# ETH3D/dataset-pipeline

Hardware: AMD Instinct MI355X
Metric: ICP correspondences/sec (higher is better)
Workload: dtype f32 (f64 accumulation); 1 GPU; ICPScanAligner 2 scans x 50000000 points, -d 0.01 (BASELINE.json configs[1] shape), one outer iteration per step; scans=2, parallelism=dp1

## Files before the change

### dataset-pipeline_amd/csrc/e3d_icp_kernels.hip

```cpp
#include <cstdlib>

#include "e3d_icp_kernels.hpp"

#pragma clang fp contract(off)

namespace e3d {

__global__ __launch_bounds__(kBlock) void k_transform_aos(const float* __restrict__ xyz,
                                                          const float* __restrict__ nrm, size_t n, Affine T,
                                                          float* __restrict__ oxyz, float* __restrict__ onrm,
                                                          float* __restrict__ bbox_partial) {
  float mn[3] = {3.402823466e+38f, 3.402823466e+38f, 3.402823466e+38f};
  float mx[3] = {-3.402823466e+38f, -3.402823466e+38f, -3.402823466e+38f};
  for (size_t i = (size_t)blockIdx.x * blockDim.x + threadIdx.x; i < n; i += (size_t)gridDim.x * blockDim.x) {
    const float x = xyz[3 * i], y = xyz[3 * i + 1], z = xyz[3 * i + 2];
    const float3 p = pcl_se3(T, x, y, z);
    oxyz[3 * i] = p.x; oxyz[3 * i + 1] = p.y; oxyz[3 * i + 2] = p.z;
    if (nrm) {
      const float3 q = pcl_so3(T, nrm[3 * i], nrm[3 * i + 1], nrm[3 * i + 2]);
      onrm[3 * i] = q.x; onrm[3 * i + 1] = q.y; onrm[3 * i + 2] = q.z;
    }
    mn[0] = fminf(mn[0], p.x); mn[1] = fminf(mn[1], p.y); mn[2] = fminf(mn[2], p.z);
    mx[0] = fmaxf(mx[0], p.x); mx[1] = fmaxf(mx[1], p.y); mx[2] = fmaxf(mx[2], p.z);
  }
// ... 1051 lines not shown
        const h8_t Aop = __builtin_bit_cast(h8_t, L.a[tile][gh][col]);
        const f16_t acc0 = __builtin_amdgcn_mfma_f32_32x32x16_f16(Aop, Bop[0], zero16, 0, 0, 0);
        if (two) {
          const f16_t acc1 = __builtin_amdgcn_mfma_f32_32x32x16_f16(Aop, Bop[1], zero16, 0, 0, 0);
          mf_process(acc0, Q[0], L, tile, gh, base, nb, P);
          mf_process(acc1, Q[1], L, tile, gh, base, nb, P);
        } else {
          mf_process(acc0, Q[0], L, tile, gh, base, nb, P);
        }
      }
      __builtin_amdgcn_fence(__ATOMIC_RELEASE, "wavefront");
      __builtin_amdgcn_wave_barrier();
      __builtin_amdgcn_fence(__ATOMIC_ACQUIRE, "wavefront");
    }

    float rd2 = r2; unsigned roi = 0u; int rpos = -1;
    const int slot_of_lane = (lane - f) & 63;
#pragma unroll
    for (int G = 0; G < 2; ++G) {
      int lb_pos = -1;
      {
        unsigned p = 0;
#pragma unroll
        for (int r = 0; r < 9; ++r) {
          if (Q[G].bt - p < rl[r]) lb_pos = (int)(rs[r] + (Q[G].bt - p));
          p += rl[r];
        }
      }
      float lb_d2 = Q[G].bd; unsigned lb_oi = Q[G].boi;
      {
        const float od2 = __shfl_xor(lb_d2, 32, 64);
        const unsigned ooi = (unsigned)__shfl_xor((int)lb_oi, 32, 64);
        const int opos = __shfl_xor(lb_pos, 32, 64);
        if (od2 < lb_d2 || (od2 == lb_d2 && ooi < lb_oi)) { lb_d2 = od2; lb_oi = ooi; lb_pos = opos; }
      }
      const float sd2 = __shfl(lb_d2, slot_of_lane & 31, 64);
      const unsigned soi = (unsigned)__shfl((int)lb_oi, slot_of_lane & 31, 64);
      const int spos = __shfl(lb_pos, slot_of_lane & 31, 64);
      if ((slot_of_lane >> 5) == G) { rd2 = sd2; roi = soi; rpos = spos; }
    }
    if ((seg >> lane) & 1ull) {
      if (rd2 < best_d2 || (rd2 == best_d2 && roi < best_oi)) { best_d2 = rd2; best_oi = roi; best_pos = rpos; }
    }
    remaining &= ~seg;
  }
  if (valid) { match_pos[pos] = best_pos; match_d2[pos] = best_d2; }
}

constexpr int kCertPerWave = 512;
template <int kCertUnroll>
__device__ __forceinline__ void nn_certify_body(const unsigned bx, const float4* __restrict__ Gsrc, size_t n, const float4* __restrict__ Gtgt,
                                                const MotionBound cum_up, float r2, float near2, int none_near, int* __restrict__ match,
                                                int* __restrict__ match2, const float* __restrict__ lbe,
                                                float* __restrict__ match_d2, unsigned* __restrict__ todo_near,
                                                unsigned* __restrict__ todo_far, unsigned* __restrict__ counts,
                                                unsigned* __restrict__ upd_counts = nullptr, double* __restrict__ upd_d2 = nullptr,
                                                unsigned* __restrict__ upd_groups = nullptr, unsigned char* __restrict__ upd_done = nullptr) {
  __shared__ unsigned s_list[2][kBlock / kWave][kCertPerWave];
  __shared__ unsigned s_cnt[2][kBlock / kWave];
  __shared__ unsigned s_base[2];
  const int lane = threadIdx.x & 63, w = threadIdx.x >> 6;
  const size_t j0 = ((size_t)bx * (kBlock / kWave) + (size_t)w) * kCertPerWave;
  unsigned cn = 0, cf = 0;
  for (int step0 = 0; step0 < kCertPerWave / kWave; step0 += kCertUnroll) {
    size_t jj[kCertUnroll];
    bool vv[kCertUnroll];
    int mm[kCertUnroll], mm2[kCertUnroll];
    float ll[kCertUnroll];
    float4 qq[kCertUnroll], c1[kCertUnroll], c2v[kCertUnroll];
#pragma unroll
    for (int u = 0; u < kCertUnroll; ++u) {
      jj[u] = j0 + (size_t)(step0 + u) * kWave + (size_t)lane;
      vv[u] = jj[u] < n;
      const size_t js = vv[u] ? jj[u] : 0;
      mm[u] = ld_stream(match + js); mm2[u] = ld_stream(match2 + js); ll[u] = ld_stream(lbe + js); qq[u] = ld_stream(Gsrc + js);
    }
#pragma unroll
    for (int u = 0; u < kCertUnroll; ++u) {
      c1[u] = Gtgt[mm[u] >= 0 ? mm[u] : 0];
      c2v[u] = Gtgt[(mm[u] >= 0 && mm2[u] >= 0) ? mm2[u] : 0];
    }
    unsigned ub_c = 0, ub_g = 0, ub_gm = 0;
    double ub_t = 0.0;
    bool ub_bad = false;
    static_assert(kCertUnroll == 4, "four steps of 64 queries = one block of the row update");
#pragma unroll
    for (int u = 0; u < kCertUnroll; ++u) {
    const size_t j = jj[u];
    const bool valid = vv[u];
    bool ok = false, near = false;
    bool swapped = false;
    float v_ok = 0.f;
    if (valid) {
      const float thr = (ll[u] - motion_up(qq[u], cum_up)) * 0.999999f;
      const float lim = thr * thr * 0.999999f;
      const int m = mm[u];
      if (m >= 0) {
        const int m2 = mm2[u];
        const float4 q = qq[u];
        const float4 c = c1[u];
        float v = sqdist_l2(q.x, q.y, q.z, c.x, c.y, c.z);
        if (m2 >= 0) {
          const float4 c2 = c2v[u];
          const float v2 = sqdist_l2(q.x, q.y, q.z, c2.x, c2.y, c2.z);
          if (v2 < v || (v2 == v && __float_as_uint(c2.w) < __float_as_uint(c.w))) {
            v = v2;
            if (thr > 0.f && v < lim && v < r2) { match[j] = m2; match2[j] = m; swapped = true; }
          }
        }
        ok = (thr > 0.f) && (v < lim) && (v < r2);
        near = v < near2;
        if (ok) { st_stream(match_d2 + j, v); v_ok = v; }
      } else {
        ok = (thr > 0.f) && (lim >= r2);
        near = none_near != 0;
        st_stream(match_d2 + j, r2);
      }
    }
    const unsigned long long fn = __ballot(valid && !ok && near), ff = __ballot(valid && !ok && !near);
    const unsigned long long below = (1ull << lane) - 1ull;
    if (valid && !ok) {
      if (near) s_list[0][w][cn + (unsigned)__popcll(fn & below)] = (unsigned)j;
      else s_list[1][w][cf + (unsigned)__popcll(ff & below)] = (unsigned)j | (mm[u] < 0 ? kListNoPartner : 0u);
    }
    cn += (unsigned)__popcll(fn); cf += (unsigned)__popcll(ff);
    if (upd_done) {
      const bool f = valid && mm[u] >= 0;
      const unsigned gc = (unsigned)__popcll(__ballot(f));
      const double gd = wave_sum((f && ok) ? (double)v_ok : 0.0);
      ub_c += gc; ub_t += gd;
      if (gc) { ++ub_g; ub_gm |= 1u << u; }
      if (__ballot(valid && (!ok || swapped))) ub_bad = true;
    }
    }
    if (upd_done) {
      const size_t blk = j0 / kBlock + (size_t)(step0 / kCertUnroll);
      if (blk < (n + kBlock - 1) / kBlock && lane == 0) {
        if (!ub_bad) { upd_counts[blk] = ub_c; upd_d2[blk] = ub_t; upd_groups[blk] = ub_g | (ub_gm << 8); }
        upd_done[blk] = ub_bad ? 0 : 1;
      }
    }
  }
  if (lane == 0) { s_cnt[0][w] = cn; s_cnt[1][w] = cf; }
  __syncthreads();
  if (threadIdx.x < 2) {
    unsigned tot = 0;
    for (int k = 0; k < kBlock / kWave; ++k) tot += s_cnt[threadIdx.x][k];
    s_base[threadIdx.x] = tot ? atomicAdd(&counts[threadIdx.x], tot) : 0u;
  }
  __syncthreads();
  unsigned bn = s_base[0], bf = s_base[1];
  for (int k = 0; k < w; ++k) { bn += s_cnt[0][k]; bf += s_cnt[1][k]; }
  for (unsigned i = (unsigned)lane; i < cn; i += kWave) todo_near[bn + i] = s_list[0][w][i];
  for (unsigned i = (unsigned)lane; i < cf; i += kWave) todo_far[bf + i] = s_list[1][w][i];
}

template <int kCertUnroll>
__global__ __launch_bounds__(kBlock) void k_nn_certify(const float4* __restrict__ Gsrc, size_t n, const float4* __restrict__ Gtgt,
                                                       MotionBound cum_up, float r2, float near2, int none_near, int* __restrict__ match,
                                                       int* __restrict__ match2, const float* __restrict__ lbe,
                                                       float* __restrict__ match_d2, unsigned* __restrict__ todo_near,
                                                       unsigned* __restrict__ todo_far, unsigned* __restrict__ counts) {
  nn_certify_body<kCertUnroll>(blockIdx.x, Gsrc, n, Gtgt, cum_up, r2, near2, none_near, match, match2, lbe, match_d2, todo_near, todo_far, counts);
}

__device__ __forceinline__ int nn_find_range(const unsigned* __restrict__ ends, int n, unsigned b) {
  int lo = 0, hi = n - 1;
  while (lo < hi) {
    const int mid = (lo + hi) >> 1;
    if (b < ends[mid]) hi = mid; else lo = mid + 1;
  }
  return __builtin_amdgcn_readfirstlane(lo);
}

__global__ __launch_bounds__(kBlock) void k_nn_certify_multi(const NnBatchDev* __restrict__ B, float r2) {
  const int p = nn_find_range(B->cert_end, B->n_pairs, blockIdx.x);
  const unsigned bx = blockIdx.x - (p ? B->cert_end[p - 1] : 0u);
  const NnPairDev& P = B->pair[p];
  nn_certify_body<4>(bx, P.Gsrc, (size_t)P.n, P.Gtgt, P.cum_up, r2, P.near2, P.none_near, P.match, P.match2, P.lbe, P.match_d2,
                     P.todo_near, P.todo_far, P.counts, P.upd_counts, P.upd_d2, P.upd_groups, P.upd_done);
}

template <int LPQ>
__global__ __launch_bounds__(kBlock) void k_nn_bounded(const float4* __restrict__ Gsrc, const unsigned* __restrict__ list,
                                                       unsigned n_list, const float4* __restrict__ Gtgt, const unsigned* __restrict__ S,
                                                       GridDesc g, InvMap im, QueryRange qr, float r2, BoundParams bp,
                                                       int* __restrict__ match, int* __restrict__ match2,
                                                       float* __restrict__ match_d2, float* __restrict__ lbe) {
  const unsigned i = (blockIdx.x * blockDim.x + threadIdx.x) / LPQ;
  const int sub = threadIdx.x % LPQ;
  if (i >= n_list) return;
  const unsigned j = list[i] & kListIndexMask;
  const float4 q = Gsrc[j];
  const int m = match[j];
  float d1 = r2;
  if (m >= 0) {
    const float4 pc = Gtgt[m];
    d1 = sqdist_l2(q.x, q.y, q.z, pc.x, pc.y, pc.z);
    const int m2 = match2[j];
    if (m2 >= 0) { const float4 pc2 = Gtgt[m2]; d1 = fminf(d1, sqdist_l2(q.x, q.y, q.z, pc2.x, pc2.y, pc2.z)); }
  }
  const float dr = sqrtf(fminf(d1, r2)) + ((m < 0) ? bp.np_extra : bp.margin);
  const float cover2 = (d1 < r2) ? fminf(dr * dr * 1.000001f, r2) : ((m < 0) ? dr * dr * 1.000001f : r2);
  const float rho = sqrtf(cover2) * bp.rho_scale + bp.rho_pad;
  const float dx = q.x - im.t[0], dy = q.y - im.t[1], dz = q.z - im.t[2];
  const float lx = im.Linv[0] * dx + im.Linv[1] * dy + im.Linv[2] * dz;
  const float ly = im.Linv[3] * dx + im.Linv[4] * dy + im.Linv[5] * dz;
  const float lz = im.Linv[6] * dx + im.Linv[7] * dy + im.Linv[8] * dz;
  const int x0 = max(cell_coord(lx - rho, g.origin[0], g.inv_cell) - qr.lo[0], 0), x1 = min(cell_coord(lx + rho, g.origin[0], g.inv_cell) - qr.lo[0], (int)qr.D[0] - 1);
  const int y0 = max(cell_coord(ly - rho, g.origin[1], g.inv_cell) - qr.lo[1], 0), y1 = min(cell_coord(ly + rho, g.origin[1], g.inv_cell) - qr.lo[1], (int)qr.D[1] - 1);
  const int z0 = max(cell_coord(lz - rho, g.origin[2], g.inv_cell) - qr.lo[2], 0), z1 = min(cell_coord(lz + rho, g.origin[2], g.inv_cell) - qr.lo[2], (int)qr.D[2] - 1);
  const float kInf = __uint_as_float(0x7f800000u);
  float cover_box2 = 0.f;
  if (x0 <= x1 && y0 <= y1 && z0 <= z1) {
    const float ux = (lx - g.origin[0]) * g.inv_cell - (float)qr.lo[0], uy = (ly - g.origin[1]) * g.inv_cell - (float)qr.lo[1],
                uz = (lz - g.origin[2]) * g.inv_cell - (float)qr.lo[2];
    float fd = kInf;
    if (x0 > 0) fd = fminf(fd, ux - (float)x0);
    if (x1 < (int)qr.D[0] - 1) fd = fminf(fd, (float)(x1 + 1) - ux);
    if (y0 > 0) fd = fminf(fd, uy - (float)y0);
    if (y1 < (int)qr.D[1] - 1) fd = fminf(fd, (float)(y1 + 1) - uy);
    if (z0 > 0) fd = fminf(fd, uz - (float)z0);
    if (z1 < (int)qr.D[2] - 1) fd = fminf(fd, (float)(z1 + 1) - uz);
    fd = fminf(fd, 4.0f);
    const float cb = fd * bp.cell_scale - bp.cell_sub;
    cover_box2 = cb > 0.f ? cb * cb : 0.f;
  }
  const float cover_all2 = fmaxf(cover2, cover_box2);
  float bd = kInf, bd2 = kInf, b3 = kInf;
  int bpos = -1, bpos2 = -1;
  bool tie = false;
  if (x0 <= x1) {
    for (int cz = z0; cz <= z1; ++cz) {
      for (int cy = y0; cy <= y1; ++cy) {
        const size_t row = ((size_t)cz * qr.D[1] + (size_t)cy) * qr.D[0];
        const unsigned s0 = S[row + (size_t)x0], s1 = S[row + (size_t)x1 + 1];
        for (unsigned p = s0 + (unsigned)sub; p < s1; p += LPQ) {
          const float4 c = Gtgt[p];
          const float d2 = sqdist_l2(q.x, q.y, q.z, c.x, c.y, c.z);
          const bool lt1 = d2 < bd, lt2 = d2 < bd2;
          b3 = fminf(b3, fmaxf(d2, bd2));
          bd2 = fminf(fmaxf(d2, bd), bd2);
          bpos2 = lt1 ? bpos : (lt2 ? (int)p : bpos2);
          bd = fminf(d2, bd);
          bpos = lt1 ? (int)p : bpos;
        }
      }
    }
  }
#pragma unroll
  for (int l = 1; l < LPQ; ++l) {
    const float obd = __shfl(bd, l, LPQ), obd2 = __shfl(bd2, l, LPQ), ob3 = __shfl(b3, l, LPQ);
    const int opos = __shfl(bpos, l, LPQ), opos2 = __shfl(bpos2, l, LPQ);
    if (sub == 0) {
#pragma unroll
      for (int t = 0; t < 2; ++t) {
        const float d2 = t == 0 ? obd : obd2;
        const int p = t == 0 ? opos : opos2;
        if (p >= 0) {
          const bool lt1 = d2 < bd, lt2 = d2 < bd2;
          b3 = fminf(b3, fmaxf(d2, bd2));
          bd2 = fminf(fmaxf(d2, bd), bd2);
          bpos2 = lt1 ? bpos : (lt2 ? p : bpos2);
          bd = fminf(d2, bd);
          bpos = lt1 ? p : bpos;
        }
      }
      b3 = fminf(b3, ob3);
    }
  }
  if (sub != 0) return;
  tie = (bd == bd2 && bd < kInf) || (bd2 == b3 && bd2 < kInf);
  if (tie) {
    bd = kInf; bd2 = kInf; b3 = kInf; bpos = -1; bpos2 = -1;
    unsigned boi = 0u, boi2 = 0u;
    for (int cz = z0; cz <= z1; ++cz) {
      for (int cy = y0; cy <= y1; ++cy) {
        const size_t row = ((size_t)cz * qr.D[1] + (size_t)cy) * qr.D[0];
        const unsigned s0 = S[row + (size_t)x0], s1 = S[row + (size_t)x1 + 1];
        for (unsigned p = s0; p < s1; ++p) {
          const float4 c = Gtgt[p];
          const float d2 = sqdist_l2(q.x, q.y, q.z, c.x, c.y, c.z);
          const unsigned oi = __float_as_uint(c.w);
          if (d2 < bd || (d2 == bd && oi < boi)) {
            b3 = fminf(b3, bd2); bd2 = bd; boi2 = boi; bpos2 = bpos; bd = d2; boi = oi; bpos = (int)p;
          } else if (d2 < bd2 || (d2 == bd2 && oi < boi2)) {
            b3 = fminf(b3, bd2); bd2 = d2; boi2 = oi; bpos2 = (int)p;
          } else {
            b3 = fminf(b3, d2);
          }
        }
      }
    }
  }
  const bool has1 = bd < r2, has2 = bd2 < r2;
  match[j] = has1 ? bpos : -1;
  match2[j] = has2 ? bpos2 : -1;
  match_d2[j] = has1 ? bd : r2;
  const float others2 = has2 ? b3 : (has1 ? bd2 : bd);
  lbe[j] = sqrtf(fminf(others2, cover_all2)) * 0.999999f + motion_lo(q, bp.lo);
}

constexpr int kHalfRuns = 18;
template <int BATCH>
__device__ __forceinline__ void nn_bounded_half_body(const unsigned bx, const float4* __restrict__ Gsrc, const unsigned* __restrict__ list,
                                                     unsigned n_list, const float4* __restrict__ Gtgt, const unsigned* __restrict__ S,
                                                     const unsigned long long* __restrict__ H8,
                                                     const GridDesc& g, const InvMap& im, const QueryRange& qr, float r2, const BoundParams& bp,
                                                     int* __restrict__ match, int* __restrict__ match2,
                                                     float* __restrict__ match_d2, float* __restrict__ lbe) {
  __shared__ unsigned s_runs[kHalfRuns][kBlock];
  __shared__ unsigned char s_len[kHalfRuns][kBlock];
  const unsigned i = bx * blockDim.x + threadIdx.x;
  if (i >= n_list) return;
  const unsigned j = list[i] & kListIndexMask;
  const float4 q = Gsrc[j];
  const int m = match[j];
  float d1 = r2;
  if (m >= 0) {
    const float4 pc = Gtgt[m];
    d1 = sqdist_l2(q.x, q.y, q.z, pc.x, pc.y, pc.z);
    const int m2 = match2[j];
    if (m2 >= 0) { const float4 pc2 = Gtgt[m2]; d1 = fminf(d1, sqdist_l2(q.x, q.y, q.z, pc2.x, pc2.y, pc2.z)); }
  }
  const float dr = sqrtf(fminf(d1, r2)) + ((m < 0) ? bp.np_extra : bp.margin);
  const float cover2 = (d1 < r2) ? fminf(dr * dr * 1.000001f, r2) : ((m < 0) ? dr * dr * 1.000001f : r2);
  const float rho = sqrtf(cover2) * bp.rho_scale + bp.rho_pad;
  const float dx = q.x - im.t[0], dy = q.y - im.t[1], dz = q.z - im.t[2];
  const float lx = im.Linv[0] * dx + im.Linv[1] * dy + im.Linv[2] * dz;
  const float ly = im.Linv[3] * dx + im.Linv[4] * dy + im.Linv[5] * dz;
  const float lz = im.Linv[6] * dx + im.Linv[7] * dy + im.Linv[8] * dz;
  const float inv_h = 2.f * g.inv_cell;
  const int NX = 2 * (int)qr.D[0], NY = 2 * (int)qr.D[1], NZ = 2 * (int)qr.D[2];
  const int FX0 = max(cell_coord(lx - rho, g.origin[0], inv_h) - 2 * qr.lo[0], 0), FX1 = min(cell_coord(lx + rho, g.origin[0], inv_h) - 2 * qr.lo[0], NX - 1);
  const int FY0 = max(cell_coord(ly - rho, g.origin[1], inv_h) - 2 * qr.lo[1], 0), FY1 = min(cell_coord(ly + rho, g.origin[1], inv_h) - 2 * qr.lo[1], NY - 1);
  const int FZ0 = max(cell_coord(lz - rho, g.origin[2], inv_h) - 2 * qr.lo[2], 0), FZ1 = min(cell_coord(lz + rho, g.origin[2], inv_h) - 2 * qr.lo[2], NZ - 1);
  const float kInf = __uint_as_float(0x7f800000u);
  float cover_box2 = 0.f;
  const bool any = FX0 <= FX1 && FY0 <= FY1 && FZ0 <= FZ1;
  if (any) {
    const float ux = (lx - g.origin[0]) * inv_h - (float)(2 * qr.lo[0]), uy = (ly - g.origin[1]) * inv_h - (float)(2 * qr.lo[1]),
                uz = (lz - g.origin[2]) * inv_h - (float)(2 * qr.lo[2]);
    float fd = kInf;
    if (FX0 > 0) fd = fminf(fd, ux - (float)FX0);
    if (FX1 < NX - 1) fd = fminf(fd, (float)(FX1 + 1) - ux);
    if (FY0 > 0) fd = fminf(fd, uy - (float)FY0);
    if (FY1 < NY - 1) fd = fminf(fd, (float)(FY1 + 1) - uy);
    if (FZ0 > 0) fd = fminf(fd, uz - (float)FZ0);
    if (FZ1 < NZ - 1) fd = fminf(fd, (float)(FZ1 + 1) - uz);
    fd = fminf(fd, 8.0f);
    const float cb = fd * (bp.cell_scale * 0.5f) - bp.cell_sub;
    cover_box2 = cb > 0.f ? cb * cb : 0.f;
  }
  const float cover_all2 = fmaxf(cover2, cover_box2);
  float bd = kInf, bd2 = kInf, b3 = kInf;
  int bpos = -1, bpos2 = -1;
  const int cx0 = FX0 >> 1, cx1 = FX1 >> 1;
  int nr = 0;
#define RUN_S(i) s_runs[(i)][threadIdx.x]
#define RUN_LEN(i) s_len[(i)][threadIdx.x]
#define RUN_E(i) (RUN_S(i) + (unsigned)RUN_LEN(i))
  if (any) {
    const int nz = FZ1 - FZ0 + 1, ny = FY1 - FY0 + 1, nx = cx1 - cx0 + 1;
    if (nz <= 3 && ny <= 3 && nx <= 2) {
      const int gz0 = FZ0 >> 1, gy0 = FY0 >> 1;
      unsigned cs[8];
      unsigned long long ce[8];
#pragma unroll
      for (int t = 0; t < 8; ++t) {
        const int gz = min(gz0 + (t >> 2), FZ1 >> 1), gy = min(gy0 + ((t >> 1) & 1), FY1 >> 1), cx = min(cx0 + (t & 1), cx1);
        const size_t lin = ((size_t)gz * qr.D[1] + (size_t)gy) * qr.D[0] + (size_t)cx;
        cs[t] = S[lin];
        ce[t] = H8[lin];
      }
      const int dz = (FZ1 >> 1) - gz0, dy = (FY1 >> 1) - gy0, dxc = cx1 - cx0;
      bool dense = false;
#pragma unroll
      for (int t = 0; t < 8; ++t)
        dense = dense || ((t >> 2) <= dz && ((t >> 1) & 1) <= dy && (t & 1) <= dxc && ce[t] == ~0ull);
      if (dense) {
        nr = -1;
      } else {
#pragma unroll
        for (int t = 0; t < 8; ++t) {
          if ((t >> 2) <= dz && ((t >> 1) & 1) <= dy && (t & 1) <= dxc) {
            const int cz2 = 2 * (gz0 + (t >> 2)), cy2 = 2 * (gy0 + ((t >> 1) & 1)), cx2 = 2 * (cx0 + (t & 1));
            const bool xa = FX0 > cx2, xb = FX1 > cx2;
            const unsigned st = cs[t], lo = (unsigned)ce[t], hi = (unsigned)(ce[t] >> 32);
#pragma unroll
            for (int zz = 0; zz < 2; ++zz)
#pragma unroll
              for (int yy = 0; yy < 2; ++yy) {
                if (cz2 + zz >= FZ0 && cz2 + zz <= FZ1 && cy2 + yy >= FY0 && cy2 + yy <= FY1) {
                  const int kb = zz * 4 + yy * 2;
                  const unsigned w = zz ? hi : lo;
                  const unsigned e_prev = kb == 0 ? 0u : (kb == 4 ? (lo >> 24) : ((w >> (8 * ((kb & 3) - 1))) & 0xFFu));
                  const unsigned e_x0 = (w >> (8 * (kb & 3))) & 0xFFu, e_x1 = (w >> (8 * ((kb & 3) + 1))) & 0xFFu;
                  const unsigned e0 = xa ? e_x0 : e_prev, e1 = xb ? e_x1 : e_x0;
                  if (e0 < e1) {
                    RUN_S(nr) = st + e0;
                    RUN_LEN(nr) = (unsigned char)(e1 - e0);
                    ++nr;
                  }
                }
              }
          }
        }
      }
    } else {
      nr = -1;
    }
  }
  if (nr > 0) {
    const unsigned uinf = 0x7f800000u;
    unsigned ud = uinf, ud2 = uinf, u3 = uinf;
    int r = 0;
    const int last = nr - 1;
    unsigned cur = RUN_S(0), end = RUN_E(0);
    while (r < nr) {
      unsigned p[BATCH];
      bool ok[BATCH];
#pragma unroll
      for (int t = 0; t < BATCH; ++t) {
        ok[t] = r < nr;
        p[t] = cur;
        const unsigned nx = cur + 1u;
        const bool sw = ok[t] && nx == end;
        r += sw ? 1 : 0;
        const int rc = min(r, last);
        const unsigned ns = RUN_S(rc), ne = ns + (unsigned)RUN_LEN(rc);
        cur = sw ? ns : (ok[t] ? nx : cur);
        end = sw ? ne : end;
      }
      float4 c4[BATCH];
#pragma unroll
      for (int t = 0; t < BATCH; ++t) c4[t] = Gtgt[p[t]];
#pragma unroll
      for (int t = 0; t < BATCH; ++t) {
        const unsigned u = ok[t] ? __float_as_uint(sqdist_l2(q.x, q.y, q.z, c4[t].x, c4[t].y, c4[t].z)) : uinf;
        const bool lt1 = u < ud, lt2 = u < ud2;
        u3 = min(u3, max(u, ud2));
        ud2 = min(max(u, ud), ud2);
        bpos2 = lt1 ? bpos : (lt2 ? (int)p[t] : bpos2);
        ud = min(u, ud);
        bpos = lt1 ? (int)p[t] : bpos;
      }
    }
    bd = __uint_as_float(ud); bd2 = __uint_as_float(ud2); b3 = __uint_as_float(u3);
  } else if (nr < 0) {
    for (int gz = FZ0 >> 1; gz <= (FZ1 >> 1); ++gz)
      for (int gy = FY0 >> 1; gy <= (FY1 >> 1); ++gy) {
        const size_t row = ((size_t)gz * qr.D[1] + (size_t)gy) * qr.D[0];
        const unsigned s0 = S[row + (size_t)cx0], s1 = S[row + (size_t)cx1 + 1];
        for (unsigned p = s0; p < s1; ++p) {
          const float4 c = Gtgt[p];
          const float d2 = sqdist_l2(q.x, q.y, q.z, c.x, c.y, c.z);
          const bool lt1 = d2 < bd, lt2 = d2 < bd2;
          b3 = fminf(b3, fmaxf(d2, bd2));
          bd2 = fminf(fmaxf(d2, bd), bd2);
          bpos2 = lt1 ? bpos : (lt2 ? (int)p : bpos2);
          bd = fminf(d2, bd);
          bpos = lt1 ? (int)p : bpos;
        }
      }
  }
  if (any && ((bd == bd2 && bd < kInf) || (bd2 == b3 && bd2 < kInf))) {
    bd = kInf; bd2 = kInf; b3 = kInf; bpos = -1; bpos2 = -1;
    unsigned boi = 0u, boi2 = 0u;
    auto exact_run = [&](unsigned s0, unsigned s1) {
      for (unsigned p = s0; p < s1; ++p) {
        const float4 c = Gtgt[p];
        const float d2 = sqdist_l2(q.x, q.y, q.z, c.x, c.y, c.z);
        const unsigned oi = __float_as_uint(c.w);
        if (d2 < bd || (d2 == bd && oi < boi)) {
          b3 = fminf(b3, bd2); bd2 = bd; boi2 = boi; bpos2 = bpos; bd = d2; boi = oi; bpos = (int)p;
        } else if (d2 < bd2 || (d2 == bd2 && oi < boi2)) {
          b3 = fminf(b3, bd2); bd2 = d2; boi2 = oi; bpos2 = (int)p;
        } else {
          b3 = fminf(b3, d2);
        }
      }
    };
    if (nr >= 0) {
      for (int r = 0; r < nr; ++r) exact_run(RUN_S(r), RUN_E(r));
    } else {
      for (int gz = FZ0 >> 1; gz <= (FZ1 >> 1); ++gz)
        for (int gy = FY0 >> 1; gy <= (FY1 >> 1); ++gy) {
          const size_t row = ((size_t)gz * qr.D[1] + (size_t)gy) * qr.D[0];
          exact_run(S[row + (size_t)cx0], S[row + (size_t)cx1 + 1]);
        }
    }
  }
#undef RUN_S
#undef RUN_E
#undef RUN_LEN
  const bool has1 = bd < r2, has2 = bd2 < r2;
  match[j] = has1 ? bpos : -1;
  match2[j] = has2 ? bpos2 : -1;
  match_d2[j] = has1 ? bd : r2;
  const float others2 = has2 ? b3 : (has1 ? bd2 : bd);
  lbe[j] = sqrtf(fminf(others2, cover_all2)) * 0.999999f + motion_lo(q, bp.lo);
}

template <int BATCH>
__global__ __launch_bounds__(kBlock) void k_nn_bounded_half(const float4* __restrict__ Gsrc, const unsigned* __restrict__ list,
                                                            unsigned n_list, const float4* __restrict__ Gtgt, const unsigned* __restrict__ S,
                                                            const unsigned long long* __restrict__ H8,
                                                            GridDesc g, InvMap im, QueryRange qr, float r2, BoundParams bp,
                                                            int* __restrict__ match, int* __restrict__ match2,
                                                            float* __restrict__ match_d2, float* __restrict__ lbe) {
  nn_bounded_half_body<BATCH>(blockIdx.x, Gsrc, list, n_list, Gtgt, S, H8, g, im, qr, r2, bp, match, match2, match_d2, lbe);
}

__global__ __launch_bounds__(kBlock) void k_nn_bounded_half_multi(const NnBatchDev* __restrict__ B, float r2) {
  const int jb = nn_find_range(B->job_end, B->n_jobs, blockIdx.x);
  const unsigned bx = blockIdx.x - (jb ? B->job_end[jb - 1] : 0u);
  const int p = __builtin_amdgcn_readfirstlane(B->job_pair[jb]);
  const NnPairDev& P = B->pair[p];
  const GridDesc g = P.g; const InvMap im = P.im; const QueryRange qr = P.qr; const BoundParams bp = P.bp;
  nn_bounded_half_body<8>(bx, P.Gsrc, B->job_list[jb], B->job_n[jb], P.Gtgt, P.S, P.H8, g, im, qr, r2, bp, P.match, P.match2,
                          P.match_d2, P.lbe);
}

template <typename KeyT>
__global__ __launch_bounds__(kBlock) void k_query_keys_multi(const NnBatchDev* __restrict__ B, float r2, KeyT* __restrict__ keys, unsigned* __restrict__ vals,
                                                             unsigned* __restrict__ counts) {
  const int p = nn_find_range(B->far_end, B->n_pairs, blockIdx.x);
  const unsigned bx = blockIdx.x - (p ? B->far_end[p - 1] : 0u);
  const NnPairDev& P = B->pair[p];
  const GridDesc g = P.g; const InvMap im = P.im; const QueryRange qr = P.qr;
  const CertParams cert = {P.bp.cell_scale, P.bp.cell_sub, P.bp.lo};
  const int shift = B->key_shift;
  const KeyT mask = (KeyT)(((KeyT)1 << shift) - (KeyT)1), hi = (KeyT)((KeyT)p << shift);
  const int flags = __builtin_amdgcn_readfirstlane(P.far_flags);
  query_keys_prune_body<KeyT>(bx, P.Gsrc, P.far_list, (size_t)P.far_n, P.occ, P.occ_stride, g, im, qr, r2, cert, keys, vals, counts, counts + 1 + p, mask, hi,
                              (flags & 2) != 0, P.match, P.match2, P.match_d2, P.lbe, flags & 1);
}

constexpr int kSeedPerThread = 4;
static_assert((unsigned)(kBlock * kSeedPerThread) == kQuerySeedBlock, "queries per block of the seeding key kernel");
template <typename KeyT, int kSeedProbes>
__global__ __launch_bounds__(kBlock) void k_query_seed_multi(const NnBatchDev* __restrict__ B, float r2, KeyT* __restrict__ keys, unsigned* __restrict__ vals,
                                                             unsigned* __restrict__ counts) {
  __shared__ unsigned s_cnt[2][kBlock / kWave][kSeedPerThread];
  __shared__ unsigned s_base[2];
  const int p = nn_find_range(B->far_end, B->n_pairs, blockIdx.x);
  const unsigned bx = blockIdx.x - (p ? B->far_end[p - 1] : 0u);
  const NnPairDev& P = B->pair[p];
  const GridDesc g = P.g; const InvMap im = P.im; const QueryRange qr = P.qr;
  const CertParams cert = {P.bp.cell_scale, P.bp.cell_sub, P.bp.lo};
  const int shift = B->key_shift;
  const KeyT key_mask = (KeyT)(((KeyT)1 << shift) - (KeyT)1), key_or = (KeyT)((KeyT)p << shift);
  const int flags = __builtin_amdgcn_readfirstlane(P.far_flags);
  const bool from_state = (flags & 1) != 0, prune = (flags & 2) != 0, seed_on = (flags & 4) != 0;
  const float4* __restrict__ Gsrc = P.Gsrc; const float4* __restrict__ Gtgt = P.Gtgt;
  const unsigned* __restrict__ list = P.far_list; const unsigned* __restrict__ occ = P.occ; const unsigned* __restrict__ S = P.S;
  const unsigned long long* __restrict__ H8 = P.H8;
  int* __restrict__ match = P.match; int* __restrict__ match2 = P.match2; float* __restrict__ match_d2 = P.match_d2; float* __restrict__ lbe = P.lbe;
  const size_t n = (size_t)P.far_n;
  const unsigned stride_w = P.occ_stride;
  const float seed2 = P.seed2;
  const int lane = threadIdx.x & 63, w = threadIdx.x >> 6;
  const size_t i0 = (size_t)bx * (kBlock * kSeedPerThread) + (size_t)w * kWave + (size_t)lane;
  KeyT kk[kSeedPerThread];
  unsigned jf[kSeedPerThread];
  float4 qq[kSeedPerThread];
  unsigned long long keyed_mask[kSeedPerThread], seeded_mask[kSeedPerThread];
#pragma unroll
  for (int u = 0; u < kSeedPerThread; ++u) {
    const size_t i = i0 + (size_t)u * kBlock;
    jf[u] = (i < n) ? (list ? list[i] : ((unsigned)i | ((from_state && match[i] < 0) ? kListNoPartner : 0u))) : 0u;
  }
#pragma unroll
  for (int u = 0; u < kSeedPerThread; ++u) qq[u] = Gsrc[jf[u] & kListIndexMask];
  unsigned wordv[kSeedPerThread];
  int bitv[kSeedPerThread];
  float bdist[kSeedPerThread];
  unsigned long long lin[kSeedPerThread];
  unsigned code[kSeedPerThread];
#pragma unroll
  for (int u = 0; u < kSeedPerThread; ++u) {
    const float4 q = qq[u];
    const float dx = q.x - im.t[0], dy = q.y - im.t[1], dz = q.z - im.t[2];
    const float lx = im.Linv[0] * dx + im.Linv[1] * dy + im.Linv[2] * dz;
    const float ly = im.Linv[3] * dx + im.Linv[4] * dy + im.Linv[5] * dz;
    const float lz = im.Linv[6] * dx + im.Linv[7] * dy + im.Linv[8] * dz;
    int cx = 0, cy = 0, cz = 0;
    bdist[u] = 2.0f;
    lin[u] = query_cell_key(q, im, g, qr, cx, cy, cz, &bdist[u]);
    code[u] = half_code(lx, ly, lz, g);
    kk[u] = ((KeyT)lin[u] & key_mask) | key_or;
    wordv[u] = 0u; bitv[u] = -1;
    if (lin[u] != kEmptyKey) {
      if (prune) {
        const int kx = cx - qr.lo[0], ky = cy - qr.lo[1], kz = cz - qr.lo[2];
        wordv[u] = occ[((size_t)kz * qr.D[1] + (size_t)ky) * stride_w + (size_t)(kx >> 5)];
        bitv[u] = kx & 31;
      }
    } else {
      bdist[u] = 2.0f;
    }
  }
  bool keep[kSeedPerThread];
  unsigned s0[kSeedPerThread], s1[kSeedPerThread];
  unsigned long long h8[kSeedPerThread];
  int mm[kSeedPerThread];
#pragma unroll
  for (int u = 0; u < kSeedPerThread; ++u) {
    const size_t i = i0 + (size_t)u * kBlock;
    const bool valid = i < n;
    keep[u] = valid && (prune ? (bitv[u] >= 0 && ((wordv[u] >> bitv[u]) & 1u)) : true);
    const bool probe = keep[u] && seed_on && lin[u] != kEmptyKey;
    const size_t l = probe ? (size_t)lin[u] : 0;
    s0[u] = S[l]; s1[u] = S[l + 1];
    h8[u] = H8[l];
    mm[u] = probe ? match[jf[u] & kListIndexMask] : -1;
    if (!probe) { s0[u] = 0u; s1[u] = 0u; }
  }
#pragma unroll
  for (int u = 0; u < kSeedPerThread; ++u) {
    const size_t i = i0 + (size_t)u * kBlock;
    const bool valid = i < n;
    const unsigned j = jf[u] & kListIndexMask;
    const float4 q = qq[u];
    if (valid && from_state && (jf[u] & kListNoPartner)) match_d2[j] = r2;
    if (valid && !keep[u]) {
      if (!(jf[u] & kListNoPartner)) {
        match[j] = -1; match_d2[j] = r2;
        if (match2) match2[j] = -1;
      }
      const float kInf = __uint_as_float(0x7f800000u);
      const float lb_out = bdist[u] * cert.cell_scale - cert.cell_sub;
      lbe[j] = fmaxf(fminf(sqrtf(kInf), lb_out), 0.0f) * 0.999999f + motion_lo(q, cert.lo);
    }
    unsigned a = s0[u], b = s1[u];
    if (h8[u] != ~0ull && b > a) {
      const unsigned c = code[u];
      const unsigned e_hi = (unsigned)(h8[u] >> (8 * c)) & 0xFFu, e_lo = c ? ((unsigned)(h8[u] >> (8 * (c - 1))) & 0xFFu) : 0u;
      if (e_hi > e_lo) { b = a + e_hi; a = a + e_lo; }
    }
    const unsigned len = b - a;
    float4 c4[kSeedProbes];
    unsigned pp[kSeedProbes];
#pragma unroll
    for (int t = 0; t < kSeedProbes; ++t) {
      const unsigned o = len > (unsigned)kSeedProbes ? ((unsigned)t * len) / (unsigned)kSeedProbes : min((unsigned)t, len ? len - 1u : 0u);
      pp[t] = a + o;
      c4[t] = Gtgt[pp[t]];
    }
    const float4 co = Gtgt[mm[u] >= 0 ? mm[u] : 0];
    const unsigned uinf = 0x7f800000u;
    unsigned ub = uinf;
    int bpos = -1;
#pragma unroll
    for (int t = 0; t < kSeedProbes; ++t) {
      const unsigned ud = len ? __float_as_uint(sqdist_l2(q.x, q.y, q.z, c4[t].x, c4[t].y, c4[t].z)) : uinf;
      bpos = ud < ub ? (int)pp[t] : bpos;
      ub = min(ud, ub);
    }
    const unsigned uo = mm[u] >= 0 ? __float_as_uint(sqdist_l2(q.x, q.y, q.z, co.x, co.y, co.z)) : uinf;
    const unsigned us = __float_as_uint(seed2);
    const bool by_old = uo < us && uo <= ub;
    const bool by_probe = !by_old && ub < us;
    if (by_probe) { match[j] = bpos; if (match2) match2[j] = -1; }
    const bool seeded = keep[u] && (by_old || by_probe);
    keyed_mask[u] = __ballot(keep[u] && !seeded);
    seeded_mask[u] = __ballot(seeded);
    if (lane == 0) { s_cnt[0][w][u] = (unsigned)__popcll(keyed_mask[u]); s_cnt[1][w][u] = (unsigned)__popcll(seeded_mask[u]); }
  }
  __syncthreads();
  if (threadIdx.x < 2) {
    const int k = threadIdx.x;
    unsigned tot = 0u;
    for (int ww = 0; ww < kBlock / kWave; ++ww)
      for (int u = 0; u < kSeedPerThread; ++u) tot += s_cnt[k][ww][u];
    s_base[k] = 0u;
    if (tot) {
      if (k == 0) { s_base[0] = atomicAdd(counts, tot); atomicAdd(counts + 1 + p, tot); }
      else s_base[1] = atomicAdd(counts + 1 + kNnBatchPairs + p, tot);
    }
  }
  __syncthreads();
  unsigned offk = s_base[0], offs = s_base[1];
  for (int ww = 0; ww < w; ++ww)
#pragma unroll
    for (int u = 0; u < kSeedPerThread; ++u) { offk += s_cnt[0][ww][u]; offs += s_cnt[1][ww][u]; }
  unsigned* __restrict__ seed_list = P.seed_list;
  const unsigned long long below = (1ull << lane) - 1ull;
#pragma unroll
  for (int u = 0; u < kSeedPerThread; ++u) {
    if ((keyed_mask[u] >> lane) & 1ull) {
      const unsigned slot = offk + (unsigned)__popcll(keyed_mask[u] & below);
      keys[slot] = kk[u];
      vals[slot] = jf[u];
    }
    if ((seeded_mask[u] >> lane) & 1ull) seed_list[offs + (unsigned)__popcll(seeded_mask[u] & below)] = jf[u] & kListIndexMask;
    offk += (unsigned)__popcll(keyed_mask[u]);
    offs += (unsigned)__popcll(seeded_mask[u]);
  }
}

__global__ __launch_bounds__(kBlock, 6) void k_nn_rows_multi(const NnBatchDev* __restrict__ B, const unsigned* __restrict__ order, float r2, int row_span) {
  const int p = nn_find_range(B->rows_end, B->n_pairs, blockIdx.x);
  const unsigned bx = blockIdx.x - (p ? B->rows_end[p - 1] : 0u);
  const NnPairDev& P = B->pair[p];
  const GridDesc g = P.g; const InvMap im = P.im; const QueryRange qr = P.qr;
  const CertParams cert = {P.bp.cell_scale, P.bp.cell_sub, P.bp.lo};
  nn_rows_body(bx, P.Gsrc, order + P.rows_off, (size_t)P.rows_n, P.Gtgt, P.S, g, im, qr, r2, row_span, cert, P.match, P.match_d2, P.lbe, P.match2);
}

__global__ __launch_bounds__(kBlock) void k_match_block_counts(const int* __restrict__ match_pos, size_t n,
                                                               unsigned* __restrict__ block_counts,
                                                               double* __restrict__ block_d2,
                                                               const float* __restrict__ match_d2) {
  const size_t j = (size_t)blockIdx.x * blockDim.x + threadIdx.x;
  const bool f = (j < n) && (ld_stream(match_pos + j) >= 0);
  const unsigned long long b = __ballot(f);
  double d = (f && match_d2) ? (double)ld_stream(match_d2 + j) : 0.0;
  d = wave_sum(d);
  __shared__ unsigned sc[kBlock / kWave];
  __shared__ double sd[kBlock / kWave];
  if ((threadIdx.x & 63) == 0) { sc[threadIdx.x >> 6] = (unsigned)__popcll(b); sd[threadIdx.x >> 6] = d; }
  __syncthreads();
  if (threadIdx.x == 0) {
    unsigned c = 0; double t = 0;
    for (int k = 0; k < kBlock / kWave; ++k) { c += sc[k]; t += sd[k]; }
    block_counts[blockIdx.x] = c; block_d2[blockIdx.x] = t;
  }
}

constexpr int kScanChunk = 256;
__device__ __forceinline__ void scan_chunk_sums_body(const unsigned bx, const unsigned* __restrict__ counts, int nblocks,
                                                     const double* __restrict__ block_d2,
                                                     unsigned long long* __restrict__ chunk_sum,
                                                     double* __restrict__ chunk_d2,
                                                     const unsigned* __restrict__ groups,
                                                     unsigned* __restrict__ chunk_groups,
                                                     unsigned* __restrict__ chunk_rewritten) {
  const int b = (int)bx * kScanChunk + threadIdx.x;
  unsigned long long c = (b < nblocks) ? counts[b] : 0ull;
  double d = (b < nblocks) ? block_d2[b] : 0.0;
  const unsigned gw = (groups && b < nblocks) ? groups[b] : 0u;
  unsigned g = gw & 0xFFu, rw = gw >> 16;
#pragma unroll
  for (int o = 32; o > 0; o >>= 1) { c += __shfl_xor(c, o, 64); d += __shfl_xor(d, o, 64); g += __shfl_xor(g, o, 64); rw += __shfl_xor(rw, o, 64); }
  __shared__ unsigned long long sc[kScanChunk / kWave];
  __shared__ double sd[kScanChunk / kWave];
  __shared__ unsigned sg[kScanChunk / kWave], sr[kScanChunk / kWave];
  if ((threadIdx.x & 63) == 0) { sc[threadIdx.x >> 6] = c; sd[threadIdx.x >> 6] = d; sg[threadIdx.x >> 6] = g; sr[threadIdx.x >> 6] = rw; }
  __syncthreads();
  if (threadIdx.x == 0) {
    unsigned long long t = 0; double td = 0; unsigned tg = 0, tr = 0;
    for (int k = 0; k < kScanChunk / kWave; ++k) { t += sc[k]; td += sd[k]; tg += sg[k]; tr += sr[k]; }
    chunk_sum[bx] = t; chunk_d2[bx] = td;
    if (chunk_groups) { chunk_groups[bx] = tg; chunk_rewritten[bx] = tr; }
  }
}

__global__ __launch_bounds__(kScanChunk) void k_scan_chunk_sums(const unsigned* __restrict__ counts, int nblocks,
                                                                const double* __restrict__ block_d2,
                                                                unsigned long long* __restrict__ chunk_sum,
                                                                double* __restrict__ chunk_d2,
                                                                const unsigned* __restrict__ groups = nullptr,
                                                                unsigned* __restrict__ chunk_groups = nullptr,
                                                                unsigned* __restrict__ chunk_rewritten = nullptr) {
  scan_chunk_sums_body(blockIdx.x, counts, nblocks, block_d2, chunk_sum, chunk_d2, groups, chunk_groups, chunk_rewritten);
}

__device__ __forceinline__ void scan_chunks_body(unsigned long long* __restrict__ chunk_sum, int nchunks, const double* __restrict__ chunk_d2,
                                                 unsigned long long* __restrict__ total, double* __restrict__ total_d2,
                                                 unsigned* __restrict__ chunk_groups, const unsigned* __restrict__ chunk_rewritten) {
  __shared__ unsigned long long s[1024];
  __shared__ double sd[1024];
  __shared__ unsigned sg[1024];
  __shared__ unsigned long long sr[1024];
  const int t = threadIdx.x, T = blockDim.x;
  const int per = (nchunks + T - 1) / T;
  const int b0 = min(nchunks, t * per), b1 = min(nchunks, b0 + per);
  unsigned long long sum = 0, rs = 0; double d = 0; unsigned gs = 0;
  for (int b = b0; b < b1; ++b) { sum += chunk_sum[b]; d += chunk_d2[b]; if (chunk_groups) { gs += chunk_groups[b]; rs += chunk_rewritten[b]; } }
  s[t] = sum; sd[t] = d; sg[t] = gs; sr[t] = rs;
  __syncthreads();
  if (t == 0) {
    unsigned long long run = 0, rr = 0; double dr = 0; unsigned gr = 0;
    for (int k = 0; k < T; ++k) {
      const unsigned long long v = s[k]; s[k] = run; run += v; dr += sd[k];
      const unsigned gv = sg[k]; sg[k] = gr; gr += gv; rr += sr[k];
    }
    *total = run; *total_d2 = dr;
    if (chunk_groups) { total[1] = gr; total[2] = rr; }
  }
  __syncthreads();
  unsigned long long run = s[t];
  unsigned grun = sg[t];
  for (int b = b0; b < b1; ++b) {
    const unsigned long long v = chunk_sum[b]; chunk_sum[b] = run; run += v;
    if (chunk_groups) { const unsigned gv = chunk_groups[b]; chunk_groups[b] = grun; grun += gv; }
  }
}

__global__ void k_scan_chunks(unsigned long long* __restrict__ chunk_sum, int nchunks, const double* __restrict__ chunk_d2,
                              unsigned long long* __restrict__ total, double* __restrict__ total_d2,
                              unsigned* __restrict__ chunk_groups = nullptr, const unsigned* __restrict__ chunk_rewritten = nullptr) {
  scan_chunks_body(chunk_sum, nchunks, chunk_d2, total, total_d2, chunk_groups, chunk_rewritten);
// ... 1031 lines not shown
```

Baseline: 6.692 billion correspondences/s.

## Rewrite bounded-half NN inner loop with buffer loads and mask-based run walking

Reworks the inner candidate loop of the bounded half-cell nearest-neighbour kernel. Run lengths are packed into 32-bit shared words, and each batch computes byte offsets for up to three consecutive runs with bitmask selects instead of serial per-element run stepping. Target points are fetched through raw buffer loads, which clamp out-of-range reads, and best-index tracking uses v_med3 and packed 2-wide float math. Other pointers are cast to global address space so the compiler emits global rather than flat loads. This adds an n_pts guard below 2^27 so the 16-byte offsets fit in 32 bits, and it depends on inline asm and on the extra padding rows in shared memory.

```diff
diff --git a/dataset-pipeline_amd/csrc/e3d_icp_kernels.hip b/dataset-pipeline_amd/csrc/e3d_icp_kernels.hip
--- a/dataset-pipeline_amd/csrc/e3d_icp_kernels.hip
+++ b/dataset-pipeline_amd/csrc/e3d_icp_kernels.hip
@@ -1377,6 +1377,25 @@
 }
 
 constexpr int kHalfRuns = 18;
+constexpr int kHalfLenWords = 6;
+struct GlobalF4 {
+  typedef float v4_t __attribute__((ext_vector_type(4)));
+  const __attribute__((address_space(1))) v4_t* p;
+  __device__ explicit GlobalF4(const float4* q) : p((const __attribute__((address_space(1))) v4_t*)q) {}
+  __device__ float4 operator[](size_t i) const { const v4_t v = p[i]; return make_float4(v.x, v.y, v.z, v.w); }
+};
+typedef float f4_t __attribute__((ext_vector_type(4)));
+constexpr int kBufferRsrcWord3 = 0x00020000;
+__device__ __forceinline__ unsigned bit_mask(unsigned m, int t) {
+  unsigned r;
+  asm("v_bfe_i32 %0, %1, %2, 1" : "=v"(r) : "v"(m), "i"(t));
+  return r;
+}
+__device__ __forceinline__ unsigned med3_u32(unsigned a, unsigned b, unsigned c) {
+  unsigned m;
+  asm("v_med3_u32 %0, %1, %2, %3" : "=v"(m) : "v"(a), "v"(b), "v"(c));
+  return m;
+}
 template <int BATCH>
 __device__ __forceinline__ void nn_bounded_half_body(const unsigned bx, const float4* __restrict__ Gsrc, const unsigned* __restrict__ list,
                                                      unsigned n_list, const float4* __restrict__ Gtgt, const unsigned* __restrict__ S,
@@ -1384,19 +1403,23 @@
                                                      const GridDesc& g, const InvMap& im, const QueryRange& qr, float r2, const BoundParams& bp,
                                                      int* __restrict__ match, int* __restrict__ match2,
                                                      float* __restrict__ match_d2, float* __restrict__ lbe) {
-  __shared__ unsigned s_runs[kHalfRuns][kBlock];
-  __shared__ unsigned char s_len[kHalfRuns][kBlock];
+  __shared__ unsigned s_runs[kHalfRuns + 2][kBlock];
+  __shared__ unsigned s_lenw[kHalfLenWords][kBlock];
   const unsigned i = bx * blockDim.x + threadIdx.x;
   if (i >= n_list) return;
-  const unsigned j = list[i] & kListIndexMask;
-  const float4 q = Gsrc[j];
-  const int m = match[j];
+#define E3D_AS1(T, ptr) ((T __attribute__((address_space(1)))*)(ptr))
+  const GlobalF4 Gt{Gtgt}, Gs{Gsrc};
+  const auto Sg = E3D_AS1(const unsigned, S);
+  const auto H8g = E3D_AS1(const unsigned long long, H8);
+  const unsigned j = E3D_AS1(const unsigned, list)[i] & kListIndexMask;
+  const float4 q = Gs[j];
+  const int m = E3D_AS1(int, match)[j];
   float d1 = r2;
   if (m >= 0) {
-    const float4 pc = Gtgt[m];
+    const float4 pc = Gt[m];
     d1 = sqdist_l2(q.x, q.y, q.z, pc.x, pc.y, pc.z);
-    const int m2 = match2[j];
-    if (m2 >= 0) { const float4 pc2 = Gtgt[m2]; d1 = fminf(d1, sqdist_l2(q.x, q.y, q.z, pc2.x, pc2.y, pc2.z)); }
+    const int m2 = E3D_AS1(int, match2)[j];
+    if (m2 >= 0) { const float4 pc2 = Gt[m2]; d1 = fminf(d1, sqdist_l2(q.x, q.y, q.z, pc2.x, pc2.y, pc2.z)); }
   }
   const float dr = sqrtf(fminf(d1, r2)) + ((m < 0) ? bp.np_extra : bp.margin);
   const float cover2 = (d1 < r2) ? fminf(dr * dr * 1.000001f, r2) : ((m < 0) ? dr * dr * 1.000001f : r2);
@@ -1431,13 +1454,17 @@
   float bd = kInf, bd2 = kInf, b3 = kInf;
   int bpos = -1, bpos2 = -1;
   const int cx0 = FX0 >> 1, cx1 = FX1 >> 1;
+  const unsigned n_pts = Sg[(size_t)qr.D[0] * qr.D[1] * qr.D[2]];
   int nr = 0;
 #define RUN_S(i) s_runs[(i)][threadIdx.x]
-#define RUN_LEN(i) s_len[(i)][threadIdx.x]
-#define RUN_E(i) (RUN_S(i) + (unsigned)RUN_LEN(i))
+#define RUN_LEN(i) ((s_lenw[(i) >> 2][threadIdx.x] >> (8 * ((i) & 3))) & 0xFFu)
+#define RUN_E(i) (RUN_S(i) + RUN_LEN(i))
   if (any) {
+#pragma unroll
+    for (int w = 0; w < kHalfLenWords; ++w) s_lenw[w][threadIdx.x] = 0u;
+    unsigned char* const len_bytes = reinterpret_cast<unsigned char*>(&s_lenw[0][0]);
     const int nz = FZ1 - FZ0 + 1, ny = FY1 - FY0 + 1, nx = cx1 - cx0 + 1;
-    if (nz <= 3 && ny <= 3 && nx <= 2) {
+    if (nz <= 3 && ny <= 3 && nx <= 2 && n_pts < (1u << 27)) {
       const int gz0 = FZ0 >> 1, gy0 = FY0 >> 1;
       unsigned cs[8];
       unsigned long long ce[8];
@@ -1445,8 +1472,8 @@
       for (int t = 0; t < 8; ++t) {
         const int gz = min(gz0 + (t >> 2), FZ1 >> 1), gy = min(gy0 + ((t >> 1) & 1), FY1 >> 1), cx = min(cx0 + (t & 1), cx1);
         const size_t lin = ((size_t)gz * qr.D[1] + (size_t)gy) * qr.D[0] + (size_t)cx;
-        cs[t] = S[lin];
-        ce[t] = H8[lin];
+        cs[t] = Sg[lin];
+        ce[t] = H8g[lin];
       }
       const int dz = (FZ1 >> 1) - gz0, dy = (FY1 >> 1) - gy0, dxc = cx1 - cx0;
       bool dense = false;
@@ -1474,7 +1501,7 @@
                   const unsigned e0 = xa ? e_x0 : e_prev, e1 = xb ? e_x1 : e_x0;
                   if (e0 < e1) {
                     RUN_S(nr) = st + e0;
-                    RUN_LEN(nr) = (unsigned char)(e1 - e0);
+                    len_bytes[4 * ((nr >> 2) * kBlock + threadIdx.x) + (nr & 3)] = (unsigned char)(e1 - e0);
                     ++nr;
                   }
                 }
@@ -1487,48 +1514,58 @@
     }
   }
   if (nr > 0) {
+    const __amdgpu_buffer_rsrc_t rsrc = __builtin_amdgcn_make_buffer_rsrc((void*)Gtgt, (short)0, (int)(16u * n_pts), kBufferRsrcWord3);
     const unsigned uinf = 0x7f800000u;
+    const f2_t nqxy = {-q.x, -q.y};
     unsigned ud = uinf, ud2 = uinf, u3 = uinf;
+    int bp16 = -16, bp16_2 = -16;
     int r = 0;
-    const int last = nr - 1;
-    unsigned cur = RUN_S(0), end = RUN_E(0);
+    unsigned k0 = 0;
     while (r < nr) {
-      unsigned p[BATCH];
-      bool ok[BATCH];
+      const unsigned lw = __builtin_amdgcn_alignbyte(s_lenw[(r >> 2) + 1][threadIdx.x], s_lenw[r >> 2][threadIdx.x], (unsigned)(r & 3));
+      const unsigned a0 = s_runs[r][threadIdx.x] + k0, a1 = s_runs[r + 1][threadIdx.x], a2 = s_runs[r + 2][threadIdx.x];
+      const int c1 = (int)((lw & 0xFFu) - k0), c2 = c1 + (int)((lw >> 8) & 0xFFu), c3 = c2 + (int)((lw >> 16) & 0xFFu);
+      const unsigned b0 = 16u * a0, b1 = 16u * (a1 - (unsigned)c1), b2 = 16u * (a2 - (unsigned)c2);
+      const unsigned m1 = __builtin_amdgcn_ubfe(~0u, 0, (unsigned)min(c1, 31)), m2 = __builtin_amdgcn_ubfe(~0u, 0, (unsigned)min(c2, 31)),
+                     m3 = __builtin_amdgcn_ubfe(~0u, 0, (unsigned)min(c3, 31));
+      unsigned off[BATCH], okm[BATCH];
 #pragma unroll
       for (int t = 0; t < BATCH; ++t) {
-        ok[t] = r < nr;
-        p[t] = cur;
-        const unsigned nx = cur + 1u;
-        const bool sw = ok[t] && nx == end;
-        r += sw ? 1 : 0;
-        const int rc = min(r, last);
-        const unsigned ns = RUN_S(rc), ne = ns + (unsigned)RUN_LEN(rc);
-        cur = sw ? ns : (ok[t] ? nx : cur);
-        end = sw ? ne : end;
-      }
-      float4 c4[BATCH];
-#pragma unroll
-      for (int t = 0; t < BATCH; ++t) c4[t] = Gtgt[p[t]];
+        const unsigned s1 = bit_mask(m1, t), s2 = bit_mask(m2, t);
+        okm[t] = bit_mask(m3, t);
+        off[t] = ((b0 & s1) | (((b1 & s2) | (b2 & ~s2)) & ~s1)) + 16u * (unsigned)t;
+      }
+      f4_t c4[BATCH];
+#pragma unroll
+      for (int t = 0; t < BATCH; ++t) c4[t] = __builtin_bit_cast(f4_t, __builtin_amdgcn_raw_buffer_load_b128(rsrc, (int)off[t], 0, 0));
 #pragma unroll
       for (int t = 0; t < BATCH; ++t) {
-        const unsigned u = ok[t] ? __float_as_uint(sqdist_l2(q.x, q.y, q.z, c4[t].x, c4[t].y, c4[t].z)) : uinf;
+        const f2_t cxy = {c4[t].x, c4[t].y};
+        const f2_t dxy = cxy + nqxy;
+        const f2_t sxy = dxy * dxy;
+        const float dz = q.z - c4[t].z;
+        const float d2 = (sxy.x + sxy.y) + dz * dz;
+        const unsigned u = (__float_as_uint(d2) & okm[t]) | (uinf & ~okm[t]);
         const bool lt1 = u < ud, lt2 = u < ud2;
-        u3 = min(u3, max(u, ud2));
-        ud2 = min(max(u, ud), ud2);
-        bpos2 = lt1 ? bpos : (lt2 ? (int)p[t] : bpos2);
+        u3 = med3_u32(u, ud2, u3);
+        ud2 = med3_u32(u, ud, ud2);
+        bp16_2 = lt1 ? bp16 : (lt2 ? (int)off[t] : bp16_2);
         ud = min(u, ud);
-        bpos = lt1 ? (int)p[t] : bpos;
-      }
-    }
+        bp16 = lt1 ? (int)off[t] : bp16;
+      }
+      const int nb = BATCH;
+      r += (c1 <= nb ? 1 : 0) + (c2 <= nb ? 1 : 0) + (c3 <= nb ? 1 : 0);
+      k0 = c3 <= nb ? 0u : (unsigned)(nb - (c2 <= nb ? c2 : (c1 <= nb ? c1 : -(int)k0)));
+    }
+    bpos = bp16 >> 4; bpos2 = bp16_2 >> 4;
     bd = __uint_as_float(ud); bd2 = __uint_as_float(ud2); b3 = __uint_as_float(u3);
   } else if (nr < 0) {
     for (int gz = FZ0 >> 1; gz <= (FZ1 >> 1); ++gz)
       for (int gy = FY0 >> 1; gy <= (FY1 >> 1); ++gy) {
         const size_t row = ((size_t)gz * qr.D[1] + (size_t)gy) * qr.D[0];
-        const unsigned s0 = S[row + (size_t)cx0], s1 = S[row + (size_t)cx1 + 1];
+        const unsigned s0 = Sg[row + (size_t)cx0], s1 = Sg[row + (size_t)cx1 + 1];
         for (unsigned p = s0; p < s1; ++p) {
-          const float4 c = Gtgt[p];
+          const float4 c = Gt[p];
           const float d2 = sqdist_l2(q.x, q.y, q.z, c.x, c.y, c.z);
           const bool lt1 = d2 < bd, lt2 = d2 < bd2;
           b3 = fminf(b3, fmaxf(d2, bd2));
@@ -1544,7 +1581,7 @@
     unsigned boi = 0u, boi2 = 0u;
     auto exact_run = [&](unsigned s0, unsigned s1) {
       for (unsigned p = s0; p < s1; ++p) {
-        const float4 c = Gtgt[p];
+        const float4 c = Gt[p];
         const float d2 = sqdist_l2(q.x, q.y, q.z, c.x, c.y, c.z);
         const unsigned oi = __float_as_uint(c.w);
         if (d2 < bd || (d2 == bd && oi < boi)) {
@@ -1562,7 +1599,7 @@
       for (int gz = FZ0 >> 1; gz <= (FZ1 >> 1); ++gz)
         for (int gy = FY0 >> 1; gy <= (FY1 >> 1); ++gy) {
           const size_t row = ((size_t)gz * qr.D[1] + (size_t)gy) * qr.D[0];
-          exact_run(S[row + (size_t)cx0], S[row + (size_t)cx1 + 1]);
+          exact_run(Sg[row + (size_t)cx0], Sg[row + (size_t)cx1 + 1]);
         }
     }
   }
@@ -1570,11 +1607,12 @@
 #undef RUN_E
 #undef RUN_LEN
   const bool has1 = bd < r2, has2 = bd2 < r2;
-  match[j] = has1 ? bpos : -1;
-  match2[j] = has2 ? bpos2 : -1;
-  match_d2[j] = has1 ? bd : r2;
+  E3D_AS1(int, match)[j] = has1 ? bpos : -1;
+  E3D_AS1(int, match2)[j] = has2 ? bpos2 : -1;
+  E3D_AS1(float, match_d2)[j] = has1 ? bd : r2;
   const float others2 = has2 ? b3 : (has1 ? bd2 : bd);
-  lbe[j] = sqrtf(fminf(others2, cover_all2)) * 0.999999f + motion_lo(q, bp.lo);
+  E3D_AS1(float, lbe)[j] = sqrtf(fminf(others2, cover_all2)) * 0.999999f + motion_lo(q, bp.lo);
+#undef E3D_AS1
 }
 
 template <int BATCH>
```

After: 6.687 billion correspondences/s (median of 4 runs). About the same (-0.1%).
